# zhangganlin/GlobalSfMpy

Hardware: AMD Instinct MI355X
Metric: edge_residuals_per_sec (higher is better)
Workload: dtype f64

## Files before the change

globalsfmpy_amd/csrc/colsort_kernels.hpp:

```cpp
#pragma once
#include "edge_math.hpp"
#include "lin_kernels.hpp"
#include "pcg_kernels.hpp"
#include "dense_assemble_kernels.hpp"

namespace gsfm {

#define GSFM_COL_RB 512
#define GSFM_COL_SUB GSFM_COL_RB
#define GSFM_COL_SLOT_BITS 9
static_assert(GSFM_COL_RB == (1 << GSFM_COL_SLOT_BITS), "row blocks of 512 rows");
#ifndef GSFM_COL_EPL
#define GSFM_COL_EPL 1
#endif
#define GSFM_COL_PAD 0xffffffffu

struct ColWg { uint32_t first_sub, n_sub, row0, part; };
struct ColLayoutDev {
  const ColWg* wg;
  const uint2* meta;
  const uint32_t* kcol;
  const uint16_t* kcnt;
  uint32_t cbits, cmax;
  uint32_t n_wg, nch;
  const uint16_t* k16;
  const uint32_t* kbase;
  const uint32_t* kdel;
};
#define GSFM_K16_CNT_ESC 7u
#define GSFM_K16_DEL_ESC 15u
__host__ __device__ constexpr uint32_t col_pack(uint32_t slot, uint32_t rowcount, uint32_t rowl) { return slot | (rowcount << GSFM_COL_SLOT_BITS) | (rowl << (2 * GSFM_COL_SLOT_BITS + 1)); }
__host__ __device__ __forceinline__ uint32_t col_slot(uint32_t y) { return y & ((1u << GSFM_COL_SLOT_BITS) - 1u); }
__host__ __device__ __forceinline__ uint32_t col_rowcount(uint32_t y) { return (y >> GSFM_COL_SLOT_BITS) & ((2u << GSFM_COL_SLOT_BITS) - 1u); }
__host__ __device__ __forceinline__ uint32_t col_rowl(uint32_t y) { return y >> (2 * GSFM_COL_SLOT_BITS + 1); }
__device__ __forceinline__ uint32_t wave_incl_scan(uint32_t x) {
  int v = (int)x;
  v += __builtin_amdgcn_update_dpp(0, v, 0x111, 0xf, 0xf, false);
  v += __builtin_amdgcn_update_dpp(0, v, 0x112, 0xf, 0xf, false);
  v += __builtin_amdgcn_update_dpp(0, v, 0x114, 0xf, 0xf, false);
  v += __builtin_amdgcn_update_dpp(0, v, 0x118, 0xf, 0xf, false);
  v += __builtin_amdgcn_update_dpp(0, v, 0x142, 0xa, 0xf, false);
  v += __builtin_amdgcn_update_dpp(0, v, 0x143, 0xc, 0xf, false);
  return (uint32_t)v;
}

__device__ __forceinline__ uint2 col_load_meta(const uint2* p) {
  uint2 v;
  v.x = __builtin_nontemporal_load(&p->x); v.y = __builtin_nontemporal_load(&p->y);
  return v;
}

struct ColMatvecArgs {
  ColLayoutDev L;
  const double2 *b0, *b1, *b2;
  const double* u;
  double* part;
  const int* done;
};
template <bool K16, typename Stop>
__device__ __forceinline__ void mv_col_body(const ColMatvecArgs& a, Stop stop_after_request) {
  constexpr int RB = GSFM_COL_RB, EPL = GSFM_COL_EPL;
  __shared__ double slots[2][EPL][3][RB];
  __shared__ uint32_t wtot[2][EPL][RB / 64];
  const ColWg w = a.L.wg[blockIdx.x];
  const uint32_t r = threadIdx.x, wave = r >> 6;
  double y0 = 0.0, y1 = 0.0, y2 = 0.0;
  uint32_t m[EPL], pos[EPL], cbase[EPL]; double2 A[EPL], B[EPL], C[EPL];
  const uint32_t cmask = (1u << a.L.cbits) - 1u, cshift = a.L.cbits + GSFM_COL_SLOT_BITS, cmax = a.L.cmax;
  auto request = [&](uint32_t s) {
#pragma unroll
    for (int k = 0; k < EPL; ++k) {
      const uint32_t sc = w.first_sub + min(s + (uint32_t)k, w.n_sub - 1);
      const size_t e = (size_t)sc * RB + r;
      pos[k] = (uint32_t)e;
      if constexpr (K16) { m[k] = __builtin_nontemporal_load(a.L.k16 + e); cbase[k] = a.L.kbase[(size_t)sc * (RB / 64) + __builtin_amdgcn_readfirstlane(wave)]; }
      else { m[k] = __builtin_nontemporal_load(a.L.kcol + e); cbase[k] = 0u; }
      A[k] = nt_load2(a.b0 + e); B[k] = nt_load2(a.b1 + e); C[k] = nt_load2(a.b2 + e);
    }
  };
  if (w.n_sub) request(0);
  if (stop_after_request()) return;
  int buf = 0;
  for (uint32_t s = 0; s < w.n_sub; s += EPL, buf ^= 1) {
    uint32_t cnt[EPL], inc[EPL];
#pragma unroll
    for (int k = 0; k < EPL; ++k) {
      uint32_t cam, pm, c;
      if constexpr (K16) {
        uint32_t dl = m[k] >> 12;
        if (dl == GSFM_K16_DEL_ESC) dl = a.L.kdel[pos[k]];
        cam = cbase[k] + wave_incl_scan(dl);
        pm = m[k] & ((1u << GSFM_COL_SLOT_BITS) - 1u);
        c = (m[k] >> GSFM_COL_SLOT_BITS) & 7u;
        if (c == GSFM_K16_CNT_ESC) c = a.L.kcnt[pos[k]];
      } else {
        cam = (m[k] & cmask) == cmask ? 0u : (m[k] & cmask); pm = (m[k] >> a.L.cbits) & ((1u << GSFM_COL_SLOT_BITS) - 1u);
        c = m[k] >> cshift;
        if (c == cmax) c = a.L.kcnt[pos[k]];
      }
      const double* um = a.u + 3 * (size_t)cam;
      const double u0 = um[0], u1 = um[1], u2 = um[2];
      slots[buf][k][0][pm] = A[k].x * u0 + A[k].y * u1 + B[k].x * u2;
      slots[buf][k][1][pm] = A[k].y * u0 + B[k].y * u1 + C[k].x * u2;
      slots[buf][k][2][pm] = B[k].x * u0 + C[k].x * u1 + C[k].y * u2;
      cnt[k] = s + (uint32_t)k < w.n_sub ? c : 0u;
      inc[k] = wave_incl_scan(cnt[k]);
      if ((r & 63u) == 63u) wtot[buf][k][wave] = inc[k];
    }
    if (s + EPL < w.n_sub) request(s + EPL);
    __syncthreads();
#pragma unroll
    for (int k = 0; k < EPL; ++k) {
      uint32_t s1 = inc[k];
      for (uint32_t v = 0; v < wave; ++v) s1 += wtot[buf][k][v];
      for (uint32_t t = s1 - cnt[k]; t < s1; ++t) { y0 += slots[buf][k][0][t]; y1 += slots[buf][k][1][t]; y2 += slots[buf][k][2][t]; }
    }
  }
  const size_t o = (size_t)w.part * RB + r, plane = (size_t)a.L.n_wg * RB;
  a.part[o] = y0; a.part[plane + o] = y1; a.part[2 * plane + o] = y2;
}
#define GSFM_K3C_THREADS GSFM_COL_RB
template <bool K16>
__global__ void __launch_bounds__(GSFM_K3C_THREADS) k_mv_col(ColMatvecArgs a) {
  if (a.done && *a.done) return;
  mv_col_body<K16>(a, [] { return false; });
}
struct ColMatvecCgArgs { ColMatvecArgs mv; Cg2Args cg; };
template <bool K16>
__global__ void __launch_bounds__(GSFM_K3C_THREADS) k_mv_col_cg(ColMatvecCgArgs aa) {
  __shared__ double lds[4];
  const Cg2Args& c = aa.cg;
  mv_col_body<K16>(aa.mv, [&]() -> bool {
    const int done = c.sc->done, iters = c.sc->iters;
    const double gamma0 = c.sc->gamma0, tol = c.sc->tol;
    const bool estop = cg_energy_stop(c.sc->einc, c.sc->esum, c.sc->etol2, iters);
    double gpart = 0.0;
    if (threadIdx.x < GSFM_BLOCK) for (int k = threadIdx.x; k < c.nb_cam; k += GSFM_BLOCK) gpart += c.part_g[(size_t)c.par * c.nb_cam + k];
    gpart = wave_sum(gpart);
    if ((threadIdx.x & 63u) == 0 && threadIdx.x < GSFM_BLOCK) lds[threadIdx.x >> 6] = gpart;
    __syncthreads();
    double gamma = 0.0;
#pragma unroll
    for (int k = 0; k < GSFM_BLOCK / 64; ++k) gamma += lds[k];
    if (done) return true;
    bool conv;
    if (c.first) {
      const double rz_abs = c.sc->rz_abs;
      conv = !(gamma > rz_abs);
      if (blockIdx.x == 0 && threadIdx.x == 0) { c.sc->gamma0 = gamma; c.sc->tol = cg_tol_with_floor(tol, rz_abs, gamma); if (conv) { c.sc->done = 1; c.sc->last_rel = 0.0; } }
    } else {
      const double rel = sqrt(gamma / gamma0);
      conv = !(rel > tol) || iters >= c.max_iters || estop;
      if (blockIdx.x == 0 && threadIdx.x == 0) { c.sc->last_rel = rel; if (conv) c.sc->done = 1; }
    }
    return conv;
  });
}
struct ColFinishArgs {
  uint32_t n_rows, row_base, nch, n_wg;
  const double* part; const double* Mblk; const double* p; const double2* q; double* y; const int* done;
  double* dot_part;
};
__global__ void __launch_bounds__(GSFM_BLOCK) k_mv_col_finish(ColFinishArgs a) {
  if (a.done && *a.done) return;
  __shared__ double lds[8];
  const uint32_t row = blockIdx.x * GSFM_BLOCK + threadIdx.x;
  double pAp = 0.0;
  if (row < a.n_rows) {
  const uint32_t blk = row / GSFM_COL_RB, r = row % GSFM_COL_RB;
  const size_t plane = (size_t)a.n_wg * GSFM_COL_RB;
  double t0 = 0.0, t1 = 0.0, t2 = 0.0;
  constexpr uint32_t FB = 8;
  for (uint32_t c0 = 0; c0 < a.nch; c0 += FB) {
    double v0[FB], v1[FB], v2[FB];
#pragma unroll
    for (uint32_t j = 0; j < FB; ++j) {
      const size_t o = ((size_t)blk * a.nch + min(c0 + j, a.nch - 1)) * GSFM_COL_RB + r;
      v0[j] = a.part[o]; v1[j] = a.part[plane + o]; v2[j] = a.part[2 * plane + o];
    }
#pragma unroll
    for (uint32_t j = 0; j < FB; ++j) if (c0 + j < a.nch) { t0 += v0[j]; t1 += v1[j]; t2 += v2[j]; }
  }
  const size_t k = a.row_base + row;
  double R[9], mp[3];
  qmat(load_q(a.q, (uint32_t)k), R);
  sym3_mulvec(a.Mblk + 6 * k, a.p + 3 * k, mp);
  const double y0 = mp[0] - (R[0] * t0 + R[1] * t1 + R[2] * t2), y1 = mp[1] - (R[3] * t0 + R[4] * t1 + R[5] * t2), y2 = mp[2] - (R[6] * t0 + R[7] * t1 + R[8] * t2);
  a.y[3 * k] = y0; a.y[3 * k + 1] = y1; a.y[3 * k + 2] = y2;
  pAp = a.p[3 * k] * y0 + a.p[3 * k + 1] * y1 + a.p[3 * k + 2] * y2;
  }
  if (a.dot_part) {
    const double t = block_sum_bcast(pAp, lds);
    if (threadIdx.x == 0) a.dot_part[blockIdx.x] = t;
  }
}

struct ColRowSArgs {
  ColLayoutDev L;
  uint32_t row_base, n_rows;
  const uint32_t* eid;
  const double2 *qr0, *qr1, *w0, *w1, *w2;
  const double* ws;
  const double2* q;
  double* s_out;
};
template <int F, int WM>
__global__ void __launch_bounds__(GSFM_BLOCK) k_col_s(ColRowSArgs a) {
  constexpr int R = ResDim<F>::R;
  const ColWg w = a.L.wg[blockIdx.x];
  for (uint32_t d = w.first_sub * GSFM_COL_SUB + threadIdx.x; d < (w.first_sub + w.n_sub) * GSFM_COL_SUB; d += GSFM_BLOCK) {
    const uint2 mt = col_load_meta(a.L.meta + d);
    if (mt.x == GSFM_COL_PAD) continue;
    const Quat qk = load_q(a.q, a.row_base + w.row0 + col_rowl(mt.y)), qm = load_q(a.q, mt.x & 0x7fffffffu);
    double2 r0, r1;
    qrel_load<WM>(a.qr0, a.qr1, d, r0, r1);
    const Quat qr = qrel_quat<WM>(r0, r1);
    const EdgeW W = load_w<WM>(a.w0, a.w1, a.w2, a.ws, d);
    double r[R];
    if (mt.x >> 31) edge_residual<F, WM>(qm, qk, qr, W, r);
    else edge_residual<F, WM>(qk, qm, qr, W, r);
    double s = 0.0;
#pragma unroll
    for (int c = 0; c < R; ++c) s += r[c] * r[c];
    a.s_out[a.eid[d]] = s;
  }
}

__global__ void __launch_bounds__(GSFM_BLOCK) k_dense_assemble_col(DenseArgs a, ColLayoutDev L) {
  for (uint32_t row = blockIdx.x * GSFM_BLOCK + threadIdx.x; row < a.n_rows; row += gridDim.x * GSFM_BLOCK) {
    for (int c = 0; c < 3; ++c) a.rcg[3 * (size_t)row + c] = 0.0;
    if (row == 0) *a.info_slot = 0.0;
    const double* M = a.Mblk + 6 * (size_t)row;
    const double m[9] = {M[0], M[1], M[2], M[1], M[3], M[4], M[2], M[4], M[5]};
    for (int r = 0; r < 3; ++r) for (int c = 0; c <= r; ++c) *dense_elem(a.A, 3 * row + r, 3 * row + c) = m[3 * r + c];
    for (int c = 0; c < 3; ++c) a.A[(((size_t)a.T * (a.T + 1) / 2) + (3 * row + c) / 32) * 1024 + (3 * row + c) % 32] = a.b[3 * (size_t)row + c];
    if (row == 0) for (uint32_t g = a.n; g < a.T * 32; ++g) *dense_elem(a.A, g, g) = 1.0;
  }
  const ColWg w = L.wg[blockIdx.x];
  const uint32_t nblk = L.n_wg / L.nch, b = w.row0 / GSFM_COL_RB;
  const uint32_t p0 = L.wg[b].first_sub * GSFM_COL_SUB;
  const ColWg wl = L.wg[(L.nch - 1) * nblk + b];
  const uint32_t p1 = (wl.first_sub + wl.n_sub) * GSFM_COL_SUB;
  for (uint32_t d = w.first_sub * GSFM_COL_SUB + threadIdx.x; d < (w.first_sub + w.n_sub) * GSFM_COL_SUB; d += GSFM_BLOCK) {
    const uint2 mt = col_load_meta(L.meta + d);
    if (mt.x == GSFM_COL_PAD) continue;
// ... 207 lines not shown
```

globalsfmpy_amd/csrc/host_common.hpp:

```cpp
#pragma once

#include <dlfcn.h>
#include <hip/hip_runtime.h>

#include <algorithm>
#include <exception>
#include <functional>
#include <stdexcept>
#include <chrono>
#include <cmath>
#include <cstdio>
#include <cstdlib>
#include <cstring>
#include <limits>
#include <sched.h>
#include <string>
#include <thread>
#include <atomic>
#include <vector>

#include "../../include/gsfm_rot.h"
#include "kernels.hpp"
#include "cov_kernels.hpp"
#include "dense_kernels.hpp"
// ... 278 lines not shown
  DevBuf<double2> h0_b, h1_b, h2_b;
  DevBuf<double> gD_b;
  int lin_set = 0;
  std::vector<uint32_t> h_cost_eid;

  DevBuf<double> x, x_trial, aa_io, active, scale, gD, Mblk, Minv, Lam, Tinv, b, D6;
  DevBuf<double2> q, q_trial;
  DevBuf<double> xcg, r, z, p, Ap, s_dir, part_g2, part_d2;
  const double* b_rhs = nullptr;
  DevBuf<double> w_gather;
  uint32_t w_tail = 0;
  DevBuf<Cg2Scalars> cg2sc;
  uint32_t coarse_want = 0, coarse_n = 0, coarse_chunk = 0;
  bool coarse_adaptive = false;
  DevBuf<double> coarseA, coarseAinv, coarse_rc, coarse_xc, coarse_scale, coarse_part;
  std::vector<double> h_coarse, h_coarse_inv;
  void* pin = nullptr;
  DevBuf<double> denseA, denseL, dense_x;
  struct Components {
    std::vector<uint32_t> comp_of;
    std::vector<uint32_t> size;
    int built_cap = -1;
    bool fresh_solve = true;
    uint32_t n_items = 0, Tmax = 0, n_dense_cams = 0, n_pcg_comps = 0;
    size_t a_words = 0;
    bool all_dense = false;
    DevBuf<int32_t> cam_item;
    DevBuf<uint32_t> cam_loc;
    DevBuf<CholBatchItem> items;
    DevBuf<double> slab, b_pcg;
    DevBuf<int> info, active;
    DevBuf<uint32_t> item_ptr, item_cams;
    DevBuf<unsigned long long> stepmax, stepprev;
    DevBuf<double> steprad;
    DevBuf<int> frozen;
    double graph_freeze = -1.0;
    hipGraphExec_t graph = nullptr;
    bool graph_lap = false;
    const void* graph_planes = nullptr;
    void drop_graph() { if (graph) (void)hipGraphExecDestroy(graph); graph = nullptr; }
    hipStream_t side = nullptr;
    hipEvent_t ev_fork = nullptr, ev_join = nullptr;
    int side_state = 0;
    void drop_side() {
      if (ev_fork) (void)hipEventDestroy(ev_fork);
      if (ev_join) (void)hipEventDestroy(ev_join);
      if (side) (void)hipStreamDestroy(side);
      side = nullptr; ev_fork = ev_join = nullptr; side_state = 0;
    }
  } comps;
  uint64_t loss_epoch = 0;
  hipGraphExec_t dense_graph = nullptr;
  bool dense_graph_lap = false;
  const void* dense_graph_planes = nullptr;
  int nb_mv = 1, mv_reps = 1;
  bool packed = false;
  bool pcg_local = false;
  DevBuf<double> b_own;
  bool component_rest = true;
  uint32_t n_components = 1;
  DevBuf<double> part_a, part_b, part_cost, part_cam, part_gauge, scal;
  DevBuf<CgScalars> cgsc;
  int nb_cam = 1, nb_cost = 1;

  DevLoss h_loss{};
  DevBuf<DevLoss> d_loss;
  DevBuf<double> tables[3];
  gsfm_loss_callback cb = nullptr;
  void* cb_user = nullptr;
  DevBuf<double> rho_ext, s_ext, w_orig;
  std::vector<double> h_s, h_rho;

  struct ColSort {
    bool active = false;
    uint32_t nch = 0, n_wg = 0;
    size_t n_pos = 0;
    DevBuf<ColWg> wg;
    DevBuf<uint2> meta;
    DevBuf<uint32_t> kcol;
    DevBuf<uint16_t> kcnt;
    uint32_t cbits = 0, cmax = 0;
    DevBuf<double> part;
    DevBuf<double> cost_part;
    bool k16_active = false;
    DevBuf<uint16_t> k16;
    DevBuf<uint32_t> kbase, kdel;
    ColLayoutDev dev() const { return ColLayoutDev{wg.p, meta.p, kcol.p, kcnt.p, cbits, cmax, n_wg, nch, k16_active ? k16.p : nullptr, kbase.p, kdel.p}; }
  } cs;

  SigmaDev sigma{};
  bool sigma_pending_cost = false, sigma_pending_lin = false;
  DevBuf<double> sigma_table, sigma_sum;

  bool have_lin = false;
  double* rec_host = nullptr;
  double* rec_dev = nullptr;
  double* mail_host = nullptr;
  double* mail_dev = nullptr;
  DevBuf<double> mail_count;
  double mail_expected = 0.0;
  int mail_state = 0;
  bool loss_staircase = false;
  bool loss_cuts_off = false;
  bool fast_lin_ok = true;
  int graph_launches = 0;
  int n_collectives = 0, n_pcg_collectives = 0, n_pcg_launched = 0;
  std::vector<double> trace;
  EventTimer timer;
};
```

globalsfmpy_amd/csrc/problem_create.hpp:

```cpp
#pragma once
#include "host_structure.hpp"

namespace {

gsfm_rot_options default_options() { gsfm_rot_options o; gsfm_rot_options_default(&o); return o; }

struct ErrorTypeInfo { int functor, wmode; bool need_cov, need_inl; };
ErrorTypeInfo classify_error_type(int32_t error_type) {
  switch (error_type) {
    case GSFM_ROT_QUATERNION_NORM:        return {F_QNORM, W_NONE, false, false};
    case GSFM_ROT_ROTATION_MAT_FNORM:     return {F_RFNORM, W_NONE, false, false};
    case GSFM_ROT_QUATERNION_COSINE:      return {F_QCOS, W_NONE, false, false};
    case GSFM_ROT_ANGLE_AXIS_COVARIANCE:  return {F_AA, W_MATRIX, true, false};
    case GSFM_ROT_ANGLE_AXIS_INLIERS:     return {F_AA, W_SCALAR, false, true};
    case GSFM_ROT_ANGLE_AXIS_COV_INLIERS: return {F_AA, W_MATRIX, true, true};
    case GSFM_ROT_ANGLE_AXIS_COVTRACE:
    case GSFM_ROT_ANGLE_AXIS_COVNORM:     return {F_AA, W_SCALAR, true, false};
    default:                              return {F_AA, W_NONE, false, false};
  }
}

template <typename EidVec>
int upload_planes(gsfm_rot_problem* P, EdgePlanes& pl, const EidVec& eid, const double* d_rel_aa) {
  pl.n = eid.size();
// ... 70 lines not shown
  if (et.need_inl && !inlier_weight) return fail(GSFM_ERR_INVALID_ARG, "this error type needs per-edge inlier weights");
  P->n_cams = n_cams; P->n_edges_in = n_edges; P->error_type = error_type;
  P->functor = et.functor;
  P->res_dim = gsfm_rot_residual_dim(error_type);
  P->param_dim = P->functor == F_AA ? 3 : 4;
  P->wmode = et.wmode;
  {
    const char* env = getenv("GSFM_LAPLACIAN");
    P->lap_capable = (P->functor == F_AA || P->functor == F_QCOS) && !(env && atoi(env) == 0);
    P->lap = P->lap_capable;
  }
  if (multi_rank) {
    P->own_begin = std::min<uint64_t>((uint64_t)shard->rank * shard->slice_width, n_cams);
    P->own_end = std::min<uint64_t>((uint64_t)(shard->rank + 1) * shard->slice_width, n_cams);
    P->n_pad = shard->slice_width * shard->world_size;
  } else { P->own_begin = 0; P->own_end = n_cams; P->n_pad = n_cams; P->shard.slice_width = n_cams; P->shard.world_size = 1; }
  P->n_rows = P->own_end - P->own_begin;
  if (hipHostMalloc(&P->pin, 512, hipHostMallocDefault) != hipSuccess) { P->pin = nullptr; (void)hipGetLastError(); }
  return 0;
}

HostStructure host_structure_input(const gsfm_rot_problem* P, uint64_t n_edges, const uint32_t* edge_i, const uint32_t* edge_j) {
  HostStructure H;
  H.n_cams = P->n_cams; H.own_begin = P->own_begin; H.own_end = P->own_end; H.n_rows = P->n_rows; H.sharded = P->sharded;
  H.n_edges = n_edges; H.edge_i = edge_i; H.edge_j = edge_j;
  return H;
}

void choose_coarse_space(gsfm_rot_problem* P, const HostStructure& H) {
  const uint32_t n_cams = H.n_cams;
  const char* env = getenv("GSFM_PCG_COARSE");
  int want = env && *env ? atoi(env) : -1;
  if (want < 0 && n_cams >= 4096) {
    double sum = 0.0; uint64_t cnt = 0;
    for (uint64_t e = 0; e < H.n_edges; e += 61) { sum += std::fabs((double)H.edge_i[e] - (double)H.edge_j[e]); ++cnt; }
    if (cnt == 0) { cnt = 1; sum = 0.0; }
    const double ratio = (double)n_cams / std::max(1.0, sum / (double)cnt);
    want = ratio >= 32.0 ? (int)std::min<uint32_t>(n_cams >= 400000 ? 128 : 64, std::max<uint32_t>(16, n_cams / 256)) : 0;
    P->coarse_adaptive = ratio < 100.0;
  }
  if (want < 0) want = 0;
  want = std::min(want, 128);
  if (want < 2 || n_cams < 4u * (uint32_t)want) want = 0;
  if (!want) return;
  P->coarse_chunk = (n_cams + want - 1) / want;
  P->coarse_want = (n_cams + P->coarse_chunk - 1) / P->coarse_chunk;
  const size_t nc = 3 * (size_t)P->coarse_want;
  const hipStream_t s = P->stream;
  if (P->coarseA.alloc(nc * nc) != hipSuccess || P->coarseAinv.alloc(nc * nc) != hipSuccess || P->coarse_rc.alloc_zeroed(nc, s) != hipSuccess ||
      P->coarse_xc.alloc_zeroed(nc + 1, s) != hipSuccess || P->coarse_scale.alloc_zeroed(2, s) != hipSuccess || P->coarse_part.alloc_zeroed(6 * (size_t)grid_for(n_cams), s) != hipSuccess) {
    P->coarseA.release(); P->coarse_want = 0; (void)hipGetLastError();
  }
}

void components_on_one_gpu(gsfm_rot_problem* P, const HostStructure& H) {
  if (P->sharded) { P->n_components = (P->shard.flags & GSFM_SHARD_DISCONNECTED) ? 2 : 1; return; }
  P->n_components = std::max<uint32_t>(1, count_components(H.n_cams, H.n_edges, H.edge_i, H.edge_j));
  if (P->n_components > 1) component_labels(H.n_cams, H.n_edges, H.edge_i, H.edge_j, &P->comps.comp_of, &P->comps.size);
}

uint32_t row_lanes(uint32_t n_rows, size_t nd) {
  const double mean_deg = n_rows ? (double)nd / n_rows : 0.0;
  if (const char* g = getenv("GSFM_ROW_LANES")) {
    const int v = atoi(g);
    if (v == 1 || v == 2 || v == 4 || v == 8 || v == 16 || v == 32 || v == 64) return (uint32_t)v;
  }
  return mean_deg >= 96 ? 64 : mean_deg >= 48 ? 32 : mean_deg >= 24 ? 16 : mean_deg >= 12 ? 8 : 4;
}

bool three_component_planes(int wmode, uint64_t n_edges) {
  const char* e = getenv("GSFM_QREL3");
  return GSFM_QREL3 != 0 && wmode == W_MATRIX && (e && *e ? atoi(e) != 0 : n_edges >= (uint64_t)1000000);
}

void upload_colsort(gsfm_rot_problem* P, ColsortHost& L, hvec<uint32_t>& col, hvec<uint32_t>& deid) {
  auto& C = P->cs;
  const hipStream_t s = P->stream;
  C.nch = L.nch; C.n_wg = (uint32_t)L.wg.size(); C.n_pos = L.n_pos; C.cbits = L.cbits; C.cmax = L.cmax;
  if (L.k16_mode != 0 && (L.k16_mode > 0 || (double)L.k16_escapes <= 0.01 * (double)L.n_pos)) {
    if (C.k16.upload(L.k16, s) == hipSuccess && C.kbase.upload(L.kbase, s) == hipSuccess && C.kdel.upload(L.kdel, s) == hipSuccess) C.k16_active = true;
    else { (void)hipGetLastError(); C.k16.release(); C.kbase.release(); C.kdel.release(); }
  }
  const bool up = C.wg.upload(L.wg, s) == hipSuccess && C.meta.upload(L.meta, s) == hipSuccess && (C.k16_active || C.kcol.upload(L.kcol, s) == hipSuccess) &&
                  C.kcnt.upload(L.kcnt, s) == hipSuccess && C.part.alloc((size_t)9 * C.n_wg * GSFM_COL_RB) == hipSuccess;
  if (sync_stream(s, "uploading the column-sorted layout") != 0 || !up) {
    (void)hipGetLastError();
    C = gsfm_rot_problem::ColSort();
    return;
  }
  if (getenv("GSFM_CREATE_TIMING")) fprintf(stderr, "gsfm create: column-sorted layout, %zu positions, 2-byte record %s (%llu escapes)\n", L.n_pos, C.k16_active ? "on" : "off", (unsigned long long)L.k16_escapes);
  col.swap(L.col); deid.swap(L.eid);
  C.active = true;
}

void choose_colsort(gsfm_rot_problem* P, HostStructure& H, int n_threads) {
  const char* env = getenv("GSFM_K3_COLSORT");
  const int mode = env && *env ? atoi(env) : -1;
  const size_t nd = H.nd();
  if (!(P->lap_capable && nd > 0 && (mode > 0 || (mode < 0 && nd >= (size_t)1000000 && P->coarse_want == 0 && P->perm.empty())))) return;
  ColsortHost L;
  if (build_colsort_host(P->n_cams, P->n_rows, H.rp, H.col, H.deid, n_threads, L)) upload_colsort(P, L, H.col, H.deid);
  if (P->cs.active) { P->coarse_want = 0; P->coarse_adaptive = false; }
}

int upload_structure(gsfm_rot_problem* P, const HostStructure& H, const double* rel_aa, size_t nd_planes) {
  {
    DevBuf<double> d_rel;
    if (d_rel.alloc(3 * H.n_edges) != hipSuccess || (H.n_edges > 0 && hipMemcpyAsync(d_rel.p, rel_aa, 24 * H.n_edges, hipMemcpyHostToDevice, P->stream) != hipSuccess))
      return fail(GSFM_ERR_HIP, "uploading the relative rotations failed");
    if (int st = upload_planes(P, P->cost, H.cost_eid, d_rel.p)) return st;
    if (int st = upload_planes(P, P->dir, H.deid, d_rel.p)) return st;
    if (int st = sync_stream(P->stream, "building the measurement planes")) return st;
  }
  if (P->cost_tiles.upload(H.tiles, P->stream) != hipSuccess) return fail(GSFM_ERR_HIP, "uploading cost tiles failed");
  P->nb_cost = (int)H.tiles.size();
  if (P->cost_idx.upload(H.cidx, P->stream) != hipSuccess || P->row_ptr.upload(H.rp, P->stream) != hipSuccess || P->col.upload(H.col, P->stream) != hipSuccess)
    return fail(GSFM_ERR_HIP, "uploading graph structure failed");
  if (P->h0.alloc(nd_planes) != hipSuccess || P->h1.alloc(nd_planes) != hipSuccess || P->h2.alloc(nd_planes) != hipSuccess)
    return fail(GSFM_ERR_HIP, "allocating normal-equation blocks failed");
  return 0;
}

int whiten_planes(gsfm_rot_problem* P, uint64_t n_edges, const double* cov6, const double* inlier_weight) {
  if (P->wmode == W_NONE) return 0;
  const ErrorTypeInfo et = classify_error_type(P->error_type);
  DevBuf<double> d_cov, d_inl;
  if (cov6 && et.need_cov && (d_cov.alloc(6 * n_edges) != hipSuccess || (n_edges && hipMemcpyAsync(d_cov.p, cov6, 48 * n_edges, hipMemcpyHostToDevice, P->stream) != hipSuccess)))
    return fail(GSFM_ERR_HIP, "upload cov6");
  if (inlier_weight && et.need_inl && (d_inl.alloc(n_edges) != hipSuccess || (n_edges && hipMemcpyAsync(d_inl.p, inlier_weight, 8 * n_edges, hipMemcpyHostToDevice, P->stream) != hipSuccess)))
    return fail(GSFM_ERR_HIP, "upload inlier weights");
  run_whiten(P, P->cost, d_cov.p, d_inl.p);
  run_whiten(P, P->dir, d_cov.p, d_inl.p);
  return sync_stream(P->stream, "whitening");
}

int alloc_camera_buffers(gsfm_rot_problem* P) {
  const size_t N = P->n_cams, NP = P->n_pad;
  P->nb_cam = grid_for(N);
  if (P->nb_cam > GSFM_MAX_PARTIALS * 64) return fail(GSFM_ERR_INVALID_ARG, "too many cameras");
  {
    const size_t rows_per_group = GSFM_BLOCK / P->G, groups = (P->n_rows + rows_per_group - 1) / rows_per_group;
    size_t max_partials = GSFM_MV_MAX_PARTIALS;
    if (P->sharded) {
      P->w_tail = 8u * (uint32_t)grid_for(P->shard.slice_width);
      max_partials = std::min<size_t>(max_partials, P->w_tail);
    }
    P->mv_reps = (int)std::max<size_t>(1, (groups + max_partials - 1) / max_partials);
    P->nb_mv = (int)std::max<size_t>(1, (groups + P->mv_reps - 1) / P->mv_reps);
  }
  bool ok = true;
  auto plain = [&](auto& buf, size_t count) { ok = ok && buf.alloc(count) == hipSuccess; };
  auto zeroed = [&](auto& buf, size_t count) { ok = ok && buf.alloc_zeroed(count, P->stream) == hipSuccess; };
  const size_t nb = (size_t)P->nb_cam;
  zeroed(P->x, 4 * N); zeroed(P->x_trial, 4 * N); zeroed(P->aa_io, 3 * N); zeroed(P->active, NP); zeroed(P->scale, 3 * N); zeroed(P->gD, 9 * NP);
  plain(P->Mblk, 6 * N); plain(P->Minv, 6 * N); plain(P->Lam, 6 * N); plain(P->Tinv, 9 * N); plain(P->b, 3 * N); plain(P->D6, 6 * N);
  plain(P->q, 2 * N); plain(P->q_trial, 2 * N);
  zeroed(P->xcg, 3 * NP); zeroed(P->r, 3 * NP); plain(P->z, 3 * N);
  zeroed(P->p, 3 * NP); zeroed(P->Ap, 3 * NP); zeroed(P->u_rot, 3 * NP);
  plain(P->part_a, nb); plain(P->part_b, nb); plain(P->part_cam, 6 * nb); plain(P->part_gauge, 9 * nb); plain(P->part_cost, (size_t)2 * P->nb_cost);
  zeroed(P->scal, SC_ALL); zeroed(P->cgsc, 1);
  zeroed(P->s_dir, 3 * N); zeroed(P->part_g2, 2 * nb); zeroed(P->part_d2, std::max(P->nb_mv, P->nb_cam)); zeroed(P->cg2sc, 1);
  if (P->sharded) zeroed(P->w_gather, ((size_t)3 * P->shard.slice_width + P->w_tail) * P->shard.world_size);
  return ok ? 0 : fail(GSFM_ERR_HIP, "allocating camera buffers failed");
}

int upload_active_mask(gsfm_rot_problem* P, const std::vector<uint32_t>& rp) {
  std::vector<double> act(P->n_pad, 0.0);
// ... 147 lines not shown
```

globalsfmpy_amd/csrc/solver_launch.hpp:

```cpp
#pragma once
#include "host_common.hpp"

namespace {

int loss_mode(const gsfm_rot_problem* P) {
  if (P->cb) return LM_SIMPLE;
  const DevLoss& L = P->h_loss;
  if (L.n == 0) return LM_SIMPLE;
  if (L.n == 1) {
    const int k = L.nodes[0].kind;
    if (k == GSFM_LOSS_MAGSAC) return (L.nodes[0].nu == 3 && !L.nodes[0].inverse) ? LM_MAGSAC : LM_PROGRAM;
    if (k == GSFM_LOSS_TRIVIAL || k == GSFM_LOSS_HUBER || k == GSFM_LOSS_SOFT_L1 || k == GSFM_LOSS_TUKEY || k == GSFM_LOSS_GEMAN_MCCLURE) return LM_SIMPLE;
  }
  return LM_PROGRAM;
}
template <typename ArgsT, template <int, int, int> class Launcher>
int dispatch(const gsfm_rot_problem* P, const ArgsT& args, int grid) {
  const int f = P->functor, w = (P->wmode == W_MATRIX && P->q3) ? W_MATRIX3 : P->wmode, l = loss_mode(P);
#define GSFM_CASE3(F, W, L) if (f == F && w == W && l == L) { Launcher<F, W, L>::go(args, grid, P->stream); return 0; }
#define GSFM_CASE(F, W) GSFM_CASE3(F, W, LM_PROGRAM) GSFM_CASE3(F, W, LM_SIMPLE) GSFM_CASE3(F, W, LM_MAGSAC)
  GSFM_CASE(F_AA, W_NONE) GSFM_CASE(F_AA, W_SCALAR) GSFM_CASE(F_AA, W_MATRIX) GSFM_CASE(F_AA, W_MATRIX3)
  GSFM_CASE(F_QCOS, W_NONE) GSFM_CASE(F_QNORM, W_NONE) GSFM_CASE(F_RFNORM, W_NONE)
#undef GSFM_CASE
#undef GSFM_CASE3
// ... 183 lines not shown
  sg->weight_zero = sg->one_over_sigma * (std::tgamma(dof_minus_one_per_two) - c.gk);
  return 0;
}

int comm_failed(gsfm_rot_problem* P, const char* what) {
  P->reset_pcg_graphs();
  P->shard.flags &= ~GSFM_SHARD_CAPTURABLE;
  return fail(GSFM_ERR_COMM, what);
}
int all_gather(gsfm_rot_problem* P, double* buf, size_t count_per_rank) {
  if (!P->sharded) return 0;
  P->n_collectives++;
  if (P->shard.all_gather(P->shard.ctx, buf, count_per_rank, (void*)P->stream) != 0) return comm_failed(P, "all_gather callback failed");
  return 0;
}
int all_reduce(gsfm_rot_problem* P, double* buf, size_t count) {
  if (!P->sharded) return 0;
  P->n_collectives++;
  if (P->shard.all_reduce_sum(P->shard.ctx, buf, count, (void*)P->stream) != 0) return comm_failed(P, "all_reduce callback failed");
  return 0;
}

enum { SC_COST = 0, SC_GMAX = 1, SC_STEP = 2 , SC_XNORM2 = 7, SC_TRIAL = 8, SC_ZL8 = 9 , SC_ZBOUND = 10 , SC_COMPBAD = 11 , SC_COMP_RADIUS = 12 , SC_DENSE_INFO = 15 , SC_N = 16,
       SC_CTL = 16 , SC_REC = 32 , SC_ALL = 96 };
enum { T_LIN = 0, T_SWEEP = 1, T_CG = 2 };

void launch_cache(gsfm_rot_problem* P, const double* x, double2* q) {
  hipLaunchKernelGGL(k_cam_cache, dim3(grid_for(P->n_cams)), dim3(GSFM_BLOCK), 0, P->stream, x, P->n_cams, P->param_dim, q);
}

template <class A> void set_rows(A& a, const gsfm_rot_problem* P) { a.n_rows = P->n_rows; a.row_base = P->own_begin; a.G = P->G; a.row_ptr = P->row_ptr.p; a.col = P->col.p; }
template <class A> void set_dir_planes(A& a, const gsfm_rot_problem* P) { a.eid = P->dir.eid.p; a.qr0 = P->dir.qr0.p; a.qr1 = P->dir.qr1.p; a.w0 = P->dir.w0.p; a.w1 = P->dir.w1.p; a.w2 = P->dir.w2.p; a.ws = P->dir.ws.p; }

int launch_row_s(gsfm_rot_problem* P, const double2* q, double* s_out, bool unit_weights) {
  if (P->cs.active) {
    ColRowSArgs ca{};
    ca.L = P->cs.dev(); ca.row_base = P->own_begin; ca.n_rows = P->n_rows; set_dir_planes(ca, P); ca.q = q; ca.s_out = s_out;
    const dim3 grid(P->cs.n_wg), blk(GSFM_BLOCK);
    if (unit_weights) return fail(GSFM_ERR_UNSUPPORTED, "unit-weight row sweep on the column-sorted layout");
    if (P->functor == F_AA && P->wmode == W_NONE) hipLaunchKernelGGL((k_col_s<F_AA, W_NONE>), grid, blk, 0, P->stream, ca);
    else if (P->functor == F_AA && P->wmode == W_SCALAR) hipLaunchKernelGGL((k_col_s<F_AA, W_SCALAR>), grid, blk, 0, P->stream, ca);
    else if (P->functor == F_AA && P->wmode == W_MATRIX && P->q3) hipLaunchKernelGGL((k_col_s<F_AA, W_MATRIX3>), grid, blk, 0, P->stream, ca);
    else if (P->functor == F_AA && P->wmode == W_MATRIX) hipLaunchKernelGGL((k_col_s<F_AA, W_MATRIX>), grid, blk, 0, P->stream, ca);
    else if (P->functor == F_QCOS) hipLaunchKernelGGL((k_col_s<F_QCOS, W_NONE>), grid, blk, 0, P->stream, ca);
    else return fail(GSFM_ERR_UNSUPPORTED, "no kernel for this error type");
    return 0;
  }
  RowSArgs ra{};
  set_rows(ra, P); set_dir_planes(ra, P); ra.q = q; ra.s_out = s_out;
  const dim3 grid(grid_for((size_t)P->n_rows * P->G)), blk(GSFM_BLOCK);
  const int f = P->functor, w = P->wmode;
#define GSFM_ROWS(F, W, U) hipLaunchKernelGGL((k_row_s<F, W, U>), grid, blk, 0, P->stream, ra)
  if (f == F_AA && w == W_SCALAR && unit_weights) GSFM_ROWS(F_AA, W_SCALAR, true);
  else if (f == F_AA && w == W_NONE) GSFM_ROWS(F_AA, W_NONE, false);
  else if (f == F_AA && w == W_SCALAR) GSFM_ROWS(F_AA, W_SCALAR, false);
  else if (f == F_AA && w == W_MATRIX && P->q3) GSFM_ROWS(F_AA, W_MATRIX3, false);
  else if (f == F_AA && w == W_MATRIX) GSFM_ROWS(F_AA, W_MATRIX, false);
  else if (f == F_QCOS) GSFM_ROWS(F_QCOS, W_NONE, false);
  else if (f == F_QNORM) GSFM_ROWS(F_QNORM, W_NONE, false);
  else if (f == F_RFNORM) GSFM_ROWS(F_RFNORM, W_NONE, false);
  else return fail(GSFM_ERR_UNSUPPORTED, "no kernel for this error type");
#undef GSFM_ROWS
  return 0;
}

CostArgs cost_args(gsfm_rot_problem* P, const double2* q) {
  CostArgs a{};
  a.tiles = P->cost_tiles.p; a.direct = P->cost_direct; a.n_cams = P->n_cams; a.n = P->cost.n; a.idx = P->cost_idx.p; a.qr0 = P->cost.qr0.p; a.qr1 = P->cost.qr1.p;
  a.w0 = P->cost.w0.p; a.w1 = P->cost.w1.p; a.w2 = P->cost.w2.p; a.ws = P->cost.ws.p; a.ws_rw = P->cost.ws.p;
  a.q = q; a.loss = P->d_loss.p; a.eid = P->cost.eid.p; a.partials = P->part_cost.p;
  return a;
}
MatvecArgs matvec_args(const gsfm_rot_problem* P, const double* Mblk, const double* p, double* y, const int* done) {
  MatvecArgs a{}; set_rows(a, P);
  a.h0 = P->h0.p; a.h1 = P->h1.p; a.h2 = P->h2.p; a.h3 = P->h3.p; a.h4 = P->h4.p; a.Mblk = Mblk; a.p = p; a.y = y; a.done = done;
  a.q = P->q_lin; a.u = P->u_rot.p;
  return a;
}
DenseArgs dense_args(const gsfm_rot_problem* P) {
  DenseArgs a{}; a.n_rows = P->n_rows; a.row_ptr = P->row_ptr.p; a.col = P->col.p; a.h0 = P->h0.p; a.h1 = P->h1.p; a.h2 = P->h2.p; a.h3 = P->h3.p; a.h4 = P->h4.p;
  a.Mblk = P->Mblk.p; a.b = P->b.p; a.q = P->q_lin; a.lap = P->lin_is_lap; a.info_slot = P->scal.p + SC_DENSE_INFO; a.rcg = P->r.p;
  return a;
}
bool chol_fused_requested() { const char* e = getenv("GSFM_CHOL_FUSED"); return e && e[0] == '1'; }

int refresh_external_rho(gsfm_rot_problem* P, const double2* q) {
  const size_t E = P->n_edges_in;
  P->h_s.resize(E); P->h_rho.resize(3 * E);
  if (P->sharded) {
    if (int st = launch_row_s(P, q, P->s_ext.p, false)) return st;
    HIPCHK(hipMemcpyAsync(P->h_s.data(), P->s_ext.p, 8 * E, hipMemcpyDeviceToHost, P->stream));
    if (int st = sync_check(P, "callback loss: read s")) return st;
    for (size_t e = 0; e < E; ++e) P->cb(P->cb_user, P->h_s[e], &P->h_rho[3 * e]);
  } else {
    CostArgs a = cost_args(P, q);
    a.s_out = P->s_ext.p; a.s_only = 1;
    if (dispatch<CostArgs, CostLauncher>(P, a, P->nb_cost)) return fail(GSFM_ERR_UNSUPPORTED, "no kernel for this error type");
    HIPCHK(hipMemcpyAsync(P->h_s.data(), P->s_ext.p, 8 * P->cost.n, hipMemcpyDeviceToHost, P->stream));
    if (int st = sync_check(P, "callback loss: read s")) return st;
    for (size_t u = 0; u < P->cost.n; ++u) P->cb(P->cb_user, P->h_s[u], &P->h_rho[3 * (size_t)P->h_cost_eid[u]]);
  }
  HIPCHK(hipMemcpyAsync(P->rho_ext.p, P->h_rho.data(), 24 * E, hipMemcpyHostToDevice, P->stream));
  return 0;
}

struct CostOutputs { double2* srho = nullptr; double2* rho12 = nullptr; double* rho1 = nullptr; double* r = nullptr; };

int launch_lin(gsfm_rot_problem* P, const double2* q, const double* go = nullptr, bool fused = false, bool spare = false);

int launch_cost(gsfm_rot_problem* P, const double2* q, int slot, const CostOutputs& out = CostOutputs(), bool reduce = true) {
  const bool sig = P->sigma_pending_cost;
  P->sigma_pending_cost = false;
  if (P->cb) {
    if (sig) {
      CostArgs a = cost_args(P, q);
      a.s_out = P->s_ext.p; a.s_only = 1; a.sigma = P->sigma; a.sigma.on = 1;
      if (dispatch<CostArgs, CostLauncher>(P, a, P->nb_cost)) return fail(GSFM_ERR_UNSUPPORTED, "no kernel for this error type");
      hipLaunchKernelGGL(k_sum_partials, dim3(1), dim3(GSFM_BLOCK), 0, P->stream, P->part_cost.p + P->nb_cost, P->nb_cost, P->sigma_sum.p);
      gsfm_loss_callback keep = P->cb;
      P->cb = nullptr;
      P->sigma_pending_lin = true;
      const int st = launch_lin(P, q);
      P->cb = keep;
      if (st) return st;
    }
    if (int st = refresh_external_rho(P, q)) return st;
  }
  CostArgs a = cost_args(P, q);
  a.rho_ext = P->cb ? P->rho_ext.p : nullptr;
  a.srho_out = out.srho; a.rho12_out = out.rho12; a.rho1_out = out.rho1; a.r_out = out.r; a.s_only = 0;
  if (sig && !P->cb) { a.sigma = P->sigma; a.sigma.on = 1; }
  const int tk = P->timer.begin(T_SWEEP);
  if (dispatch<CostArgs, CostLauncher>(P, a, P->nb_cost)) return fail(GSFM_ERR_UNSUPPORTED, "no kernel for this error type");
  P->timer.end(tk);
  if (reduce) hipLaunchKernelGGL(k_sum_partials, dim3(1), dim3(GSFM_BLOCK), 0, P->stream, P->part_cost.p, P->nb_cost, P->scal.p + slot);
  if (sig && !P->cb) hipLaunchKernelGGL(k_sum_partials, dim3(1), dim3(GSFM_BLOCK), 0, P->stream, P->part_cost.p + P->nb_cost, P->nb_cost, P->sigma_sum.p);
  return all_reduce(P, P->scal.p + slot, 1);
}

bool trial_lin_supported(const gsfm_rot_problem* P) {
  const char* e = getenv("GSFM_TRIAL_LIN");
  if (e && *e && atoi(e) == 0) return false;
  if (!P->h0_b.p || !P->cs.cost_part.p || P->sharded || P->cb || !P->cs.active || !P->lap || P->sigma_pending_cost || P->sigma_pending_lin || !k2_fast_path(P)) return false;
  const int w = (P->wmode == W_MATRIX && P->q3) ? W_MATRIX3 : P->wmode;
  return col_lin_cost_kernel(P->functor, w, loss_mode(P));
}

int launch_lin(gsfm_rot_problem* P, const double2* q, const double* go, bool fused, bool spare) {
  if (fused && !trial_lin_supported(P)) return fail(GSFM_ERR_UNSUPPORTED, "fused trial evaluation without its preconditions");
  if (P->cb) { if (int st = refresh_external_rho(P, q)) return st; }
  LinArgs a{};
  set_rows(a, P); set_dir_planes(a, P); a.ws_rw = P->dir.ws.p; a.q = q; a.loss = P->d_loss.p; a.rho_ext = P->cb ? P->rho_ext.p : nullptr; a.fast_ok = k2_fast_path(P) ? 1 : 0; a.go = go;
  if (P->sigma_pending_lin) { a.sigma = P->sigma; a.sigma.on = 1; P->sigma_pending_lin = false; }
  if (!P->lap && !P->h3.p && (P->h3.alloc(P->dir.n) != hipSuccess || P->h4.alloc(P->dir.n) != hipSuccess)) return fail(GSFM_ERR_HIP, "allocating the general normal-equation blocks failed");
  a.h0 = P->h0.p; a.h1 = P->h1.p; a.h2 = P->h2.p; a.h3 = P->h3.p; a.h4 = P->h4.p; a.gD = P->gD.p; a.lap = P->lap;
  if (spare) { a.h0 = P->h0_b.p; a.h1 = P->h1_b.p; a.h2 = P->h2_b.p; a.gD = P->gD_b.p; }
  else { P->lin_is_lap = P->lap; P->q_lin = q; }
  const int tk = P->timer.begin(T_LIN);
  if (P->cs.active) {
    ColLinArgs ca{};
    ca.lin = a; ca.L = P->cs.dev(); ca.part = P->cs.part.p; ca.cost_part = fused ? P->cs.cost_part.p : nullptr;
    if (dispatch<ColLinArgs, ColLinLauncher>(P, ca, (int)P->cs.n_wg)) return fail(GSFM_ERR_UNSUPPORTED, "no kernel for this error type");
    const bool body = col_lin_body_frame(P->functor, loss_mode(P) != LM_PROGRAM && !a.rho_ext && a.fast_ok);
    hipLaunchKernelGGL(k_lin_col_finish, dim3(grid_for(P->n_rows)), dim3(GSFM_BLOCK), 0, P->stream, P->n_rows, P->own_begin, P->cs.nch, P->cs.n_wg, (const double*)P->cs.part.p, a.gD,
                       body ? q : (const double2*)nullptr);
  } else if (dispatch<LinArgs, LinLauncher>(P, a, grid_for((size_t)P->n_rows * P->G))) return fail(GSFM_ERR_UNSUPPORTED, "no kernel for this error type");
  P->timer.end(tk);
  if (spare) return 0;
  P->have_lin = true;
  return all_gather(P, P->gD.p, (size_t)P->shard.slice_width * 9);
}

void accept_trial_lin(gsfm_rot_problem* P) {
  std::swap(P->h0.p, P->h0_b.p); std::swap(P->h1.p, P->h1_b.p); std::swap(P->h2.p, P->h2_b.p); std::swap(P->gD.p, P->gD_b.p);
  P->lin_set ^= 1;
  P->lin_is_lap = P->lap; P->q_lin = P->q.p;
  P->have_lin = true;
}

void launch_prep(gsfm_rot_problem* P, const gsfm_rot_options& o, double radius, bool init_scale, const double* radius_dev = nullptr, bool reduce = true) {
  PrepArgs a{};
  a.radius_dev = radius_dev;
  a.n = P->n_cams; a.param_dim = P->param_dim; a.x = P->x.p; a.gD = P->gD.p; a.scale = P->scale.p;
  a.init_scale = init_scale; a.jacobi_scaling = o.jacobi_scaling; a.radius = radius; a.min_diag = o.min_lm_diagonal; a.max_diag = o.max_lm_diagonal;
  a.Mblk = P->Mblk.p; a.Minv = P->Minv.p; a.Lam = P->Lam.p; a.Tinv = P->Tinv.p; a.b = P->b.p; a.gmax_partials = P->part_cam.p;
  hipLaunchKernelGGL(k_cam_prep, dim3(P->nb_cam), dim3(GSFM_BLOCK), 0, P->stream, a);
  if (reduce) {
    hipLaunchKernelGGL(k_max_partials, dim3(1), dim3(GSFM_BLOCK), 0, P->stream, P->part_cam.p, P->nb_cam, P->scal.p + SC_GMAX);
    double* part = P->part_cam.p + (size_t)5 * P->nb_cam;
    hipLaunchKernelGGL(k_cam_bound, dim3(P->nb_cam), dim3(GSFM_BLOCK), 0, P->stream, (const double*)P->Minv.p, (const double*)P->Tinv.p, (const double*)P->active.p, P->n_cams, part);
    hipLaunchKernelGGL(k_max_partials, dim3(1), dim3(GSFM_BLOCK), 0, P->stream, (const double*)part, P->nb_cam, P->scal.p + SC_ZBOUND);
  }
}

void enqueue_mv_col(gsfm_rot_problem* P, const double* Mblk, const double* p, double* y, const int* done, double* dot_part, const Cg2Args* cg = nullptr) {
  auto& c = P->cs;
  ColMatvecArgs m{};
  m.L = c.dev(); m.b0 = P->h0.p; m.b1 = P->h1.p; m.b2 = P->h2.p; m.u = P->u_rot.p; m.part = c.part.p; m.done = cg ? nullptr : done;
  const dim3 grid(c.n_wg), blk(GSFM_K3C_THREADS);
  if (cg) {
    const ColMatvecCgArgs cm{m, *cg};
    if (c.k16_active) hipLaunchKernelGGL(k_mv_col_cg<true>, grid, blk, 0, P->stream, cm);
    else hipLaunchKernelGGL(k_mv_col_cg<false>, grid, blk, 0, P->stream, cm);
  } else if (c.k16_active) hipLaunchKernelGGL(k_mv_col<true>, grid, blk, 0, P->stream, m);
  else hipLaunchKernelGGL(k_mv_col<false>, grid, blk, 0, P->stream, m);
  ColFinishArgs f{};
  f.n_rows = P->n_rows; f.row_base = P->own_begin; f.nch = c.nch; f.n_wg = c.n_wg; f.part = c.part.p; f.Mblk = Mblk; f.p = p; f.q = P->q_lin; f.y = y; f.done = done; f.dot_part = dot_part;
  hipLaunchKernelGGL(k_mv_col_finish, dim3(grid_for(P->n_rows)), dim3(GSFM_BLOCK), 0, P->stream, f);
}

int launch_matvec(gsfm_rot_problem* P, const double* Mblk, const double* p, double* y, const int* done, double* dot_part = nullptr, bool* dot_done = nullptr) {
  if (dot_done) *dot_done = false;
  if (P->cs.active) {
    if (P->sharded) dot_part = nullptr; else if (dot_part) *dot_done = true;
    enqueue_mv_col(P, Mblk, p, y, done, dot_part);
    return P->pcg_local ? 0 : all_gather(P, y, (size_t)P->shard.slice_width * 3);
  }
  const MatvecArgs a = matvec_args(P, Mblk, p, y, done);
  if (P->lin_is_lap) hipLaunchKernelGGL(k_matvec<true>, dim3(grid_for((size_t)P->n_rows * P->G)), dim3(GSFM_BLOCK), 0, P->stream, a);
  else hipLaunchKernelGGL(k_matvec<false>, dim3(grid_for((size_t)P->n_rows * P->G)), dim3(GSFM_BLOCK), 0, P->stream, a);
  return P->pcg_local ? 0 : all_gather(P, y, (size_t)P->shard.slice_width * 3);
}

}
```

Measured before the change: 8.547 billion.

## Fuse column matvec finish into main kernel via last-arriver per row block

The column-sorted matvec now publishes its partial sums with atomic stores, and the last workgroup for each 512-row block (found with an arrival counter) performs the finish reduction, the block-diagonal update and the pAp dot partials itself. This removes the separate k_mv_col_finish launch and its extra pass over the partials in the non-CG, unsharded case. In exchange it adds atomics and a vmcnt wait to every workgroup, and the finish work is serialized onto one workgroup per block. An env var keeps the separate-kernel path available.

```diff
diff --git a/globalsfmpy_amd/csrc/colsort_kernels.hpp b/globalsfmpy_amd/csrc/colsort_kernels.hpp
--- a/globalsfmpy_amd/csrc/colsort_kernels.hpp
+++ b/globalsfmpy_amd/csrc/colsort_kernels.hpp
@@ -12,6 +12,9 @@
 static_assert(GSFM_COL_RB == (1 << GSFM_COL_SLOT_BITS), "row blocks of 512 rows");
 #ifndef GSFM_COL_EPL
 #define GSFM_COL_EPL 1
+#endif
+#ifndef GSFM_COL_FIN_FB
+#define GSFM_COL_FIN_FB 3
 #endif
 #define GSFM_COL_PAD 0xffffffffu
 
@@ -50,14 +53,77 @@
   return v;
 }
 
+struct ColFinishArgs {
+  uint32_t n_rows, row_base, nch, n_wg;
+  const double* part; const double* Mblk; const double* p; const double2* q; double* y; const int* done;
+  double* dot_part;
+};
+__device__ __forceinline__ double dot3_mid(double a0, double b0, double a1, double b1, double a2, double b2) { return fma(a2, b2, fma(a0, b0, a1 * b1)); }
+__device__ __forceinline__ double dot3_first(double a0, double b0, double a1, double b1, double a2, double b2) { return fma(a2, b2, fma(a1, b1, a0 * b0)); }
+__device__ __forceinline__ void qmat_fin(const Quat& q, double* R) {
+  const double tx = 2.0 * q.x, ty = 2.0 * q.y, tz = 2.0 * q.z;
+  const double twx = tx * q.w, twy = ty * q.w, twz = tz * q.w, tyy = ty * q.y, tzz = tz * q.z;
+  R[0] = 1.0 - fma(ty, q.y, tzz); R[1] = fma(ty, q.x, -twz);      R[2] = fma(tz, q.x, twy);
+  R[3] = fma(ty, q.x, twz);       R[4] = 1.0 - fma(tx, q.x, tzz); R[5] = fma(tz, q.y, -twx);
+  R[6] = fma(tz, q.x, -twy);      R[7] = fma(tz, q.y, twx);       R[8] = 1.0 - fma(tx, q.x, tyy);
+}
+template <uint32_t FB>
+__device__ __forceinline__ double mv_col_finish_row(const ColFinishArgs& a, uint32_t row) {
+  const uint32_t blk = row / GSFM_COL_RB, r = row % GSFM_COL_RB;
+  const size_t plane = (size_t)a.n_wg * GSFM_COL_RB, k = a.row_base + row;
+  const Quat qk = load_q(a.q, (uint32_t)k);
+  double M[6], pk[3];
+#pragma unroll
+  for (int c = 0; c < 6; ++c) M[c] = a.Mblk[6 * k + c];
+#pragma unroll
+  for (int c = 0; c < 3; ++c) pk[c] = a.p[3 * k + c];
+  double t0 = 0.0, t1 = 0.0, t2 = 0.0;
+  for (uint32_t c0 = 0; c0 < a.nch; c0 += FB) {
+    double v0[FB], v1[FB], v2[FB];
+#pragma unroll
+    for (uint32_t j = 0; j < FB; ++j) {
+      const size_t o = ((size_t)blk * a.nch + min(c0 + j, a.nch - 1)) * GSFM_COL_RB + r;
+      v0[j] = a.part[o]; v1[j] = a.part[plane + o]; v2[j] = a.part[2 * plane + o];
+    }
+#pragma unroll
+    for (uint32_t j = 0; j < FB; ++j) if (c0 + j < a.nch) { t0 += v0[j]; t1 += v1[j]; t2 += v2[j]; }
+  }
+  double R[9];
+  qmat_fin(qk, R);
+  const double mp0 = dot3_mid(M[0], pk[0], M[1], pk[1], M[2], pk[2]), mp1 = dot3_mid(M[1], pk[0], M[3], pk[1], M[4], pk[2]), mp2 = dot3_mid(M[2], pk[0], M[4], pk[1], M[5], pk[2]);
+  const double y0 = mp0 - dot3_first(R[0], t0, R[1], t1, R[2], t2), y1 = mp1 - dot3_mid(R[3], t0, R[4], t1, R[5], t2), y2 = mp2 - dot3_mid(R[6], t0, R[7], t1, R[8], t2);
+  a.y[3 * k] = y0; a.y[3 * k + 1] = y1; a.y[3 * k + 2] = y2;
+  return dot3_mid(pk[0], y0, pk[1], y1, pk[2], y2);
+}
+
+__device__ __forceinline__ void col_publish(double* p, double v) { __hip_atomic_store(p, v, __ATOMIC_RELAXED, __HIP_MEMORY_SCOPE_AGENT); }
+__device__ __forceinline__ bool col_block_last_arriver(uint32_t* counter, uint32_t nch, uint32_t* lds_flag) {
+  asm volatile("s_waitcnt vmcnt(0)" ::: "memory");
+  __syncthreads();
+  if (threadIdx.x == 0) {
+    const uint32_t ticket = __hip_atomic_fetch_add(counter, 1u, __ATOMIC_RELAXED, __HIP_MEMORY_SCOPE_AGENT);
+    const bool last = ticket == nch - 1;
+    if (last) {
+      __hip_atomic_store(counter, 0u, __ATOMIC_RELAXED, __HIP_MEMORY_SCOPE_AGENT);
+      __builtin_amdgcn_fence(__ATOMIC_ACQUIRE, "agent");
+      asm volatile("s_waitcnt vmcnt(0)" ::: "memory");
+    }
+    *lds_flag = last ? 1u : 0u;
+  }
+  __syncthreads();
+  return *lds_flag != 0u;
+}
+
 struct ColMatvecArgs {
   ColLayoutDev L;
   const double2 *b0, *b1, *b2;
   const double* u;
   double* part;
   const int* done;
+  uint32_t* arrive;
+  ColFinishArgs fin;
 };
-template <bool K16, typename Stop>
+template <bool K16, bool FIN, typename Stop>
 __device__ __forceinline__ void mv_col_body(const ColMatvecArgs& a, Stop stop_after_request) {
   constexpr int RB = GSFM_COL_RB, EPL = GSFM_COL_EPL;
   __shared__ double slots[2][EPL][3][RB];
@@ -117,20 +183,39 @@
     }
   }
   const size_t o = (size_t)w.part * RB + r, plane = (size_t)a.L.n_wg * RB;
-  a.part[o] = y0; a.part[plane + o] = y1; a.part[2 * plane + o] = y2;
+  if (!FIN || !a.arrive) { a.part[o] = y0; a.part[plane + o] = y1; a.part[2 * plane + o] = y2; return; }
+  col_publish(a.part + o, y0); col_publish(a.part + plane + o, y1); col_publish(a.part + 2 * plane + o, y2);
+  __shared__ uint32_t last;
+  const uint32_t blk = w.row0 / RB;
+  if (!col_block_last_arriver(a.arrive + blk, a.L.nch, &last)) return;
+  const uint32_t row = w.row0 + r;
+  double pAp = 0.0;
+  if (row < a.fin.n_rows) pAp = mv_col_finish_row<GSFM_COL_FIN_FB>(a.fin, row);
+  if (a.fin.dot_part) {
+    double* lds = &slots[0][0][0][0];
+    pAp = wave_sum(pAp);
+    if ((r & 63u) == 0) lds[wave] = pAp;
+    __syncthreads();
+    if ((r & (GSFM_BLOCK - 1)) == 0 && (r == 0 || w.row0 + GSFM_BLOCK < a.fin.n_rows)) {
+      const double* l = lds + (r / GSFM_BLOCK) * (GSFM_BLOCK / 64);
+      double t = 0;
+      for (int k = 0; k < GSFM_BLOCK / 64; ++k) t += l[k];
+      a.fin.dot_part[2 * blk + r / GSFM_BLOCK] = t;
+    }
+  }
 }
 #define GSFM_K3C_THREADS GSFM_COL_RB
 template <bool K16>
 __global__ void __launch_bounds__(GSFM_K3C_THREADS) k_mv_col(ColMatvecArgs a) {
   if (a.done && *a.done) return;
-  mv_col_body<K16>(a, [] { return false; });
+  mv_col_body<K16, true>(a, [] { return false; });
 }
 struct ColMatvecCgArgs { ColMatvecArgs mv; Cg2Args cg; };
 template <bool K16>
 __global__ void __launch_bounds__(GSFM_K3C_THREADS) k_mv_col_cg(ColMatvecCgArgs aa) {
   __shared__ double lds[4];
   const Cg2Args& c = aa.cg;
-  mv_col_body<K16>(aa.mv, [&]() -> bool {
+  mv_col_body<K16, false>(aa.mv, [&]() -> bool {
     const int done = c.sc->done, iters = c.sc->iters;
     const double gamma0 = c.sc->gamma0, tol = c.sc->tol;
     const bool estop = cg_energy_stop(c.sc->einc, c.sc->esum, c.sc->etol2, iters);
@@ -156,11 +241,6 @@
     return conv;
   });
 }
-struct ColFinishArgs {
-  uint32_t n_rows, row_base, nch, n_wg;
-  const double* part; const double* Mblk; const double* p; const double2* q; double* y; const int* done;
-  double* dot_part;
-};
 __global__ void __launch_bounds__(GSFM_BLOCK) k_mv_col_finish(ColFinishArgs a) {
   if (a.done && *a.done) return;
   __shared__ double lds[8];
diff --git a/globalsfmpy_amd/csrc/host_common.hpp b/globalsfmpy_amd/csrc/host_common.hpp
--- a/globalsfmpy_amd/csrc/host_common.hpp
+++ b/globalsfmpy_amd/csrc/host_common.hpp
@@ -384,6 +384,8 @@
     uint32_t cbits = 0, cmax = 0;
     DevBuf<double> part;
     DevBuf<double> cost_part;
+    DevBuf<uint32_t> arrive;
+    uint32_t n_blk() const { return nch ? n_wg / nch : 0; }
     bool k16_active = false;
     DevBuf<uint16_t> k16;
     DevBuf<uint32_t> kbase, kdel;
diff --git a/globalsfmpy_amd/csrc/problem_create.hpp b/globalsfmpy_amd/csrc/problem_create.hpp
--- a/globalsfmpy_amd/csrc/problem_create.hpp
+++ b/globalsfmpy_amd/csrc/problem_create.hpp
@@ -176,7 +176,8 @@
     else { (void)hipGetLastError(); C.k16.release(); C.kbase.release(); C.kdel.release(); }
   }
   const bool up = C.wg.upload(L.wg, s) == hipSuccess && C.meta.upload(L.meta, s) == hipSuccess && (C.k16_active || C.kcol.upload(L.kcol, s) == hipSuccess) &&
-                  C.kcnt.upload(L.kcnt, s) == hipSuccess && C.part.alloc((size_t)9 * C.n_wg * GSFM_COL_RB) == hipSuccess;
+                  C.kcnt.upload(L.kcnt, s) == hipSuccess && C.part.alloc((size_t)9 * C.n_wg * GSFM_COL_RB) == hipSuccess &&
+                  C.arrive.alloc_zeroed(C.n_blk(), s) == hipSuccess;
   if (sync_stream(s, "uploading the column-sorted layout") != 0 || !up) {
     (void)hipGetLastError();
     C = gsfm_rot_problem::ColSort();
diff --git a/globalsfmpy_amd/csrc/solver_launch.hpp b/globalsfmpy_amd/csrc/solver_launch.hpp
--- a/globalsfmpy_amd/csrc/solver_launch.hpp
+++ b/globalsfmpy_amd/csrc/solver_launch.hpp
@@ -289,6 +289,7 @@
   a.Mblk = P->Mblk.p; a.b = P->b.p; a.q = P->q_lin; a.lap = P->lin_is_lap; a.info_slot = P->scal.p + SC_DENSE_INFO; a.rcg = P->r.p;
   return a;
 }
+bool col_finish_separate(const gsfm_rot_problem* P) { const char* e = getenv("GSFM_COL_FINISH"); return P->sharded || !P->cs.arrive.p || (e && !strcmp(e, "separate")); }
 bool chol_fused_requested() { const char* e = getenv("GSFM_CHOL_FUSED"); return e && e[0] == '1'; }
 
 int refresh_external_rho(gsfm_rot_problem* P, const double2* q) {
@@ -402,8 +403,12 @@
 
 void enqueue_mv_col(gsfm_rot_problem* P, const double* Mblk, const double* p, double* y, const int* done, double* dot_part, const Cg2Args* cg = nullptr) {
   auto& c = P->cs;
+  ColFinishArgs f{};
+  f.n_rows = P->n_rows; f.row_base = P->own_begin; f.nch = c.nch; f.n_wg = c.n_wg; f.part = c.part.p; f.Mblk = Mblk; f.p = p; f.q = P->q_lin; f.y = y; f.done = done; f.dot_part = dot_part;
+  const bool separate = cg || col_finish_separate(P);
   ColMatvecArgs m{};
   m.L = c.dev(); m.b0 = P->h0.p; m.b1 = P->h1.p; m.b2 = P->h2.p; m.u = P->u_rot.p; m.part = c.part.p; m.done = cg ? nullptr : done;
+  if (!separate) { m.arrive = c.arrive.p; m.fin = f; }
   const dim3 grid(c.n_wg), blk(GSFM_K3C_THREADS);
   if (cg) {
     const ColMatvecCgArgs cm{m, *cg};
@@ -411,9 +416,7 @@
     else hipLaunchKernelGGL(k_mv_col_cg<false>, grid, blk, 0, P->stream, cm);
   } else if (c.k16_active) hipLaunchKernelGGL(k_mv_col<true>, grid, blk, 0, P->stream, m);
   else hipLaunchKernelGGL(k_mv_col<false>, grid, blk, 0, P->stream, m);
-  ColFinishArgs f{};
-  f.n_rows = P->n_rows; f.row_base = P->own_begin; f.nch = c.nch; f.n_wg = c.n_wg; f.part = c.part.p; f.Mblk = Mblk; f.p = p; f.q = P->q_lin; f.y = y; f.done = done; f.dot_part = dot_part;
-  hipLaunchKernelGGL(k_mv_col_finish, dim3(grid_for(P->n_rows)), dim3(GSFM_BLOCK), 0, P->stream, f);
+  if (separate) hipLaunchKernelGGL(k_mv_col_finish, dim3(grid_for(P->n_rows)), dim3(GSFM_BLOCK), 0, P->stream, f);
 }
 
 int launch_matvec(gsfm_rot_problem* P, const double* Mblk, const double* p, double* y, const int* done, double* dot_part = nullptr, bool* dot_done = nullptr) {
```

After: 8.682 billion, median of 6. +1.6%, better.
